# Jabruson/FDN-TIP2025

Measured on AMD Instinct MI355X. Metric: images/sec, FDN (LPNet->FDN forward) 1280x720 bs=8 fp32, higher is better.
Workload: dtype f32; 1 GPU; BASELINE.json configs[1]: FDN 1280x720 (padded 1280x736) batch=8 per GPU fp32; global_batch=8, parallelism=batch-shard x1, weights=synthetic (tamed 0.03) FDN + real LPNet, hip_streams=1, rccl_ranks=1, hip_graph=True, fdsa_full=False, fdsa_pair=False, no_tail_pin=False, tail_pin_l2=False, narrow_pipe=False, unfused_mlps=False, stats_launches=False, resample_upsample=False, aff_resized=False

## Files before the change

fdn-tip2025_amd/csrc/fdsa_tail.hpp:

```cpp
#pragma once
#include "common.hpp"

namespace {

constexpr int TL_SC1 = 16;

template <bool FULL, typename T>
__device__ __forceinline__ T tl_sq_acc(T q, T dl, bool live) {
#pragma clang fp contract(off)
    const T p = dl * dl;
    if constexpr (FULL) return q + p;
    else return q + (live ? p : T(0.f));
}

__host__ __device__ constexpr int tl_image_floats(int SH, int MT) { return ((6 * 2 * SH + 3 * 2 * SH * (MT * 32 + 1) + 255) / 256) * 256; }

__host__ __device__ constexpr int tl_image_floats_px1_c(int SH, int MT) { return 512 + 3 * ((SH + 7) / 8) * MT * 3 * 64 * 4; }
struct TailIo {
    const float* scr;
    const float* res;
    float* y;
    float* stats_out;
    int E, N, W, ty0, tx0;
    unsigned P;
    float* h;
    int Hd;
    int h_bf16;
    unsigned* ring_flag;
    int* ring_cnt;
};
__device__ __forceinline__ void tl_ring_release(const TailIo& io) {
    if (io.ring_flag && (threadIdx.x & 63) == 0) {
        if (__hip_atomic_fetch_add(io.ring_cnt, 1, __ATOMIC_RELAXED, __HIP_MEMORY_SCOPE_WORKGROUP) == 3)
            __hip_atomic_store(io.ring_flag, 0u, __ATOMIC_RELAXED, __HIP_MEMORY_SCOPE_AGENT);
    }
}

template <int SH, bool PIN = false, int NT = 3, bool FULL = false>
__device__ __forceinline__ void fdsa_tail_px2(const TailIo& io, const float* lds, const float* lds_pin = nullptr) {
    typedef fdn_f32x2 T;
    typedef fdn_f32x16 f32x16;
    constexpr int E2 = 2 * SH, WS = 33;
    const float* tg = lds;
    const float* tb = lds + 3 * E2;
    const float* Wl = lds + 6 * E2;
    const int E = io.E, N = io.N;
    const unsigned P = io.P, P4 = P * 4u;
    const int lane = threadIdx.x & 63, wave = threadIdx.x >> 6, kh = lane >> 5, ln = lane & 31;
    const int row = 2 * wave + (ln >> 4), col = 2 * (ln & 15);
    const bool ok = io.tx0 + col < io.W;
    const unsigned pix = (unsigned)((io.ty0 + row) * io.W + io.tx0 + col);
    constexpr unsigned PI = 1024u;
    const rsrc_t rg[3] = {mk_rsrc(io.scr, (unsigned)E * PI), mk_rsrc(io.scr + (long)E * 256, (unsigned)E * PI),
                          mk_rsrc(io.scr + (long)2 * E * 256, (unsigned)E * PI)};
    const rsrc_t rv = mk_rsrc(io.scr + (long)3 * E * 256, (unsigned)E * PI);
    const unsigned voff = kh * PI + (unsigned)(row * 32 + col) * 4u;
    const float invE = 1.0f / (float)E;

    T vv[SH], oa[SH], ob2[SH];
#pragma unroll
    for (int s = 0; s < SH; ++s) {
        vv[s] = bload2<TL_SC1>(rv, voff, (unsigned)(2 * s) * PI);
        oa[s] = bload2<TL_SC1>(rg[0], voff, (unsigned)(2 * s) * PI);
    }
    const unsigned nb4 = (unsigned)N * P4;
    const rsrc_t ro = mk_rsrc(io.y, nb4);
    const rsrc_t rr = mk_rsrc(io.res ? io.res : io.y, io.res ? nb4 : 0u);
    const unsigned vo = ok ? (4u * kh * P + pix) * 4u : 0x80000000u;
    T rres[16];
    f32x16 acc[2];
#pragma unroll
    for (int v = 0; v < 2; ++v)
#pragma unroll
        for (int r = 0; r < 16; ++r) acc[v][r] = 0.f;

#pragma unroll
    for (int g = 0; g < 3; ++g) {
        T* cur = (g & 1) ? ob2 : oa;
        if (g < 2) {
            T* nxt = (g & 1) ? oa : ob2;
#pragma unroll
            for (int s = 0; s < SH; ++s) nxt[s] = bload2<TL_SC1>(rg[g + 1], voff, (unsigned)(2 * s) * PI);
        }
        T m = 0.f;
#pragma unroll
        for (int s = 0; s < SH; ++s) m += cur[s];
        m = xsum32(m) * invE;
        T q = 0.f;
#pragma unroll
        for (int s = 0; s < SH; ++s) {
            const T dl = cur[s] - m;
            q = tl_sq_acc<FULL>(q, dl, 2 * s + kh < E);
        }
        const T rs = rsqrt_eps(xsum32(q) * invE);
#pragma unroll
        for (int s = 0; s < SH; ++s) {
            asm volatile("" ::: "memory");
            const int e = 2 * s + kh;
            cur[s] = ((cur[s] - m) * rs * tg[g * E2 + e] + tb[g * E2 + e]) * vv[s];
        }
        if (g == 2) {
            tl_ring_release(io);
#pragma unroll
            for (int r = 0; r < 16; ++r) {
                const fdn_u32x2 u = __builtin_amdgcn_raw_buffer_load_b64(rr, vo, (unsigned)((r & 3) + 8 * (r >> 2)) * P4, 0);
                rres[r] = T{__uint_as_float(u.x), __uint_as_float(u.y)};
            }
        }
#pragma unroll
        for (int s = 0; s < SH; ++s) {
            const float wa = Wl[(g * E2 + 2 * s + kh) * WS + ln];
            acc[0] = __builtin_amdgcn_mfma_f32_32x32x2f32(wa, cur[s].x, acc[0], 0, 0, 0);
            acc[1] = __builtin_amdgcn_mfma_f32_32x32x2f32(wa, cur[s].y, acc[1], 0, 0, 0);
        }
    }
    T outv[16];
    T sm = 0.f;
#pragma unroll
    for (int r = 0; r < 16; ++r) {
        const int nrow = (r & 3) + 8 * (r >> 2);
        T o = T{acc[0][r], acc[1][r]};
        o += rres[r];
        __builtin_amdgcn_raw_buffer_store_b64(fdn_u32x2{__float_as_uint(o.x), __float_as_uint(o.y)}, ro, vo, (unsigned)nrow * P4, 0);
        outv[r] = (FULL || nrow + 4 * kh < N) ? o : T(0.f);
        sm += outv[r];
    }
    if (io.stats_out || PIN) {
        T sq = 0.f;
        const T mean = xsum32(sm) / (float)N;
#pragma unroll
        for (int r = 0; r < 16; ++r) {
            const T dl = outv[r] - mean;
            sq = tl_sq_acc<FULL>(sq, dl, (r & 3) + 8 * (r >> 2) + 4 * kh < N);
        }
        const T rstd = rsqrt_eps(xsum32(sq) / (float)N);
        if (io.stats_out && kh == 0) {
            const rsrc_t rs_ = mk_rsrc(io.stats_out, 2u * P4);
            const unsigned vs = ok ? pix * 4u : 0x80000000u;
            __builtin_amdgcn_raw_buffer_store_b64(fdn_u32x2{__float_as_uint(mean.x), __float_as_uint(mean.y)}, rs_, vs, 0u, 0);
            __builtin_amdgcn_raw_buffer_store_b64(fdn_u32x2{__float_as_uint(rstd.x), __float_as_uint(rstd.y)}, rs_, vs, P4, 0);
        }
        if constexpr (PIN) {
            fdn_u32x4 Bf[2][2][3];
#pragma unroll
            for (int c = 0; c < 2; ++c) {
                const float sa = c ? rstd.y : rstd.x, sb = -(c ? mean.y : mean.x) * sa;
                float xn[16];
#pragma unroll
                for (int r = 0; r < 16; ++r) xn[r] = fmaf(c ? outv[r].y : outv[r].x, sa, sb);
#pragma unroll
                for (int ks = 0; ks < 2; ++ks) {
                    float v[8];
#pragma unroll
                    for (int b4 = 0; b4 < 4; ++b4) {
                        const auto sw = __builtin_amdgcn_permlane32_swap(__float_as_uint(xn[8 * ks + b4]), __float_as_uint(xn[8 * ks + 4 + b4]), false, false);
                        v[b4] = __uint_as_float(sw[0]);
                        v[4 + b4] = __uint_as_float(sw[1]);
                    }
#pragma unroll
                    for (int j = 0; j < 4; ++j) {
                        unsigned p1, p2, p3;
                        fdn_split3(v[2 * j], v[2 * j + 1], p1, p2, p3);
                        Bf[c][ks][0][j] = p1, Bf[c][ks][1][j] = p2, Bf[c][ks][2][j] = p3;
                    }
                }
            }
            const fdn_u32x4* wpin = reinterpret_cast<const fdn_u32x4*>(lds_pin) + lane;
            const float* bpin = lds_pin + NT * 2 * 3 * 64 * 4;
            const rsrc_t rh = mk_rsrc(io.h, (unsigned)io.Hd * P4);
            const unsigned vh = ok ? (4u * kh * P + pix) * 4u : 0x80000000u;
#pragma unroll
            for (int t = 0; t < NT; ++t) {
                f32x16 ah[2];
#pragma unroll
                for (int g = 0; g < 4; ++g) {
                    const float4 bv = *reinterpret_cast<const float4*>(&bpin[t * 32 + 8 * g + 4 * kh]);
#pragma unroll
                    for (int c = 0; c < 2; ++c) ah[c][4 * g] = bv.x, ah[c][4 * g + 1] = bv.y, ah[c][4 * g + 2] = bv.z, ah[c][4 * g + 3] = bv.w;
                }
#pragma unroll
                for (int ks = 0; ks < 2; ++ks) {
                    const fdn_u32x4 a3[3] = {wpin[((t * 2 + ks) * 3 + 0) * 64], wpin[((t * 2 + ks) * 3 + 1) * 64], wpin[((t * 2 + ks) * 3 + 2) * 64]};
                    ah[0] = fdn_mfma_split6(a3, Bf[0][ks], ah[0]);
                    ah[1] = fdn_mfma_split6(a3, Bf[1][ks], ah[1]);
                }
                if (io.h_bf16) {
                    const rsrc_t rhb = mk_rsrc(io.h, (unsigned)io.Hd * P * 2u);
                    const unsigned vhb = ok ? (4u * kh * P + pix) * 2u : 0x80000000u;
#pragma unroll
                    for (int r = 0; r < 16; ++r)
                        __builtin_amdgcn_raw_buffer_store_b32(pack_bf16(ah[0][r], ah[1][r]), rhb, vhb, (unsigned)(t * 32 + (r & 3) + 8 * (r >> 2)) * P * 2u, 0);
                } else {
#pragma unroll
                    for (int r = 0; r < 16; ++r)
                        __builtin_amdgcn_raw_buffer_store_b64(fdn_u32x2{__float_as_uint(ah[0][r]), __float_as_uint(ah[1][r])}, rh, vh,
                                                              (unsigned)(t * 32 + (r & 3) + 8 * (r >> 2)) * P4, 0);
                }
            }
        }
    }
}

#define FDN_TAIL_FN __forceinline__
typedef __attribute__((address_space(3))) const float* lds_cf;
typedef __attribute__((address_space(3))) const fdn_u32x4* lds_cu4;
template <int SH, int MT, bool FULL = false, bool PIN = false, int NT = 6>
__device__ FDN_TAIL_FN void fdsa_tail_px1(const TailIo& io, lds_cf tg, lds_cf tb, lds_cu4 W0, lds_cu4 W1, const float* gimg) {
    typedef fdn_f32x16 f32x16;
    constexpr int E2 = 2 * SH, NQ = (SH + 7) / 8;
    const int E = io.E, N = io.N;
    const unsigned P = io.P, P4 = P * 4u;
    const int lane = threadIdx.x & 63, wave = threadIdx.x >> 6, kh = lane >> 5, ln = lane & 31;
    constexpr unsigned PI = 1024u;
    const rsrc_t rg[3] = {mk_rsrc(io.scr, (unsigned)E * PI), mk_rsrc(io.scr + (long)E * 256, (unsigned)E * PI),
                          mk_rsrc(io.scr + (long)2 * E * 256, (unsigned)E * PI)};
    const rsrc_t rv = mk_rsrc(io.scr + (long)3 * E * 256, (unsigned)E * PI);
    const rsrc_t rw2 = mk_rsrc(gimg + 512 + 2 * NQ * MT * 3 * 64 * 4, (unsigned)(NQ * MT * 3 * 64) * 16u);
    const float invE = 1.0f / (float)E;
    const unsigned nb4 = (unsigned)N * P4;
    const rsrc_t ro = mk_rsrc(io.y, nb4);
    const rsrc_t rr = mk_rsrc(io.res ? io.res : io.y, io.res ? nb4 : 0u);
    const bool ok = io.tx0 + ln < io.W;

    float vv[SH], buf[2][SH];
    auto voff_of = [&](int rnd) { return kh * PI + (unsigned)((2 * wave + rnd) * 32 + ln) * 4u; };
    {
        const unsigned voff = voff_of(0);
        unsigned PIl = PI;
        asm volatile("" : "+s"(PIl));
#pragma unroll
        for (int s = 0; s < SH; ++s) {
            vv[s] = bload<TL_SC1>(rv, voff, (unsigned)(2 * s) * PIl);
            buf[0][s] = bload<TL_SC1>(rg[0], voff, (unsigned)(2 * s) * PIl);
        }
    }
#pragma unroll
    for (int rnd = 0; rnd < 2; ++rnd) {
        unsigned P4l = P4;
        asm volatile("" : "+s"(P4l));
        int khl = kh;
        asm volatile("" : "+v"(khl));
        const unsigned voff = voff_of(rnd);
        const unsigned pix = (unsigned)((io.ty0 + 2 * wave + rnd) * io.W + io.tx0 + ln);
        const unsigned vo = ok ? (4u * kh * P + pix) * 4u : 0x80000000u;
        f32x16 acc[MT];
#pragma unroll
        for (int mt = 0; mt < MT; ++mt)
#pragma unroll
            for (int r = 0; r < 16; ++r) acc[mt][r] = 0.f;
        float rres[MT][16];
#pragma unroll
        for (int g = 0; g < 3; ++g) {
            float* cur = buf[(rnd + g) & 1];
            float* nxt = buf[(rnd + g + 1) & 1];
            unsigned PIl = PI;
            asm volatile("" : "+s"(PIl));
            if (g < 2) {
#pragma unroll
                for (int s = 0; s < SH; ++s) nxt[s] = bload<TL_SC1>(rg[g + 1], voff, (unsigned)(2 * s) * PIl);
            }
// ... 153 lines not shown
```

fdn-tip2025_amd/csrc/patchfft.hip:

```cpp
#include "patch_fft.hpp"
#include "fdsa_tail.hpp"
#include <type_traits>

namespace {

constexpr int HS = 65 + 2;
constexpr int HALO = (TH + 2) * (TW + 2);
constexpr int HPT = (HALO + 255) / 256;

__device__ __forceinline__ void halo_offsets(int H, int W, int y0, int x0, unsigned (&goff)[HPT], int (&slot)[HPT]) {
#pragma unroll
    for (int i = 0; i < HPT; ++i) {
        const int idx = threadIdx.x + 256 * i;
        const int rr = idx / (TW + 2), cc = idx - rr * (TW + 2);
        const int y = y0 - 1 + rr, x = x0 - 1 + cc;
        const bool ok = idx < HALO && y >= 0 && y < H && x >= 0 && x < W;
        goff[i] = ok ? (unsigned)(y * W + x) * 4u : OOB;
        slot[i] = idx < HALO ? rr * HS + cc : (TH + 2) * HS;
    }
}
__device__ __forceinline__ void halo_fetch(rsrc_t r, unsigned plane_off, const unsigned (&goff)[HPT], float (&v)[HPT]) {
#pragma unroll
    for (int i = 0; i < HPT; ++i) v[i] = bload(r, goff[i], plane_off);
}
// ... 419 lines not shown
            }
            fft8<true>(z);
            constexpr float sc = 1.0f / 64.0f;
#pragma unroll
            for (int i = 0; i < 8; ++i) S[pj * PS + kx * KXS + i] = make_float2(z[i].x * sc, z[i].y * sc);
        }
        __syncthreads();

        if (more) build_filter();
        {
            float2 xk[5];
#pragma unroll
            for (int kx = 0; kx < 5; ++kx) xk[kx] = S[patch * PS + kx * KXS + rr];
            float r[8];
            irfft8_row(xk, r);
            float sp[8];
            second_conv(sp);
#pragma unroll
            for (int j = 0; j < 8; ++j) r[j] += sp[j];
            st_store8<OBF>(r, rout, ooff, (unsigned)__builtin_amdgcn_readfirstlane((int)((unsigned)c * hwo)));
        }
        __syncthreads();
    }
}


constexpr int FT_H = 8, FT_W = 32;
constexpr int FHW = FT_W + 2, FHH = FT_H + 2;
constexpr int FHP = FHH * FHW;
constexpr int FNS = (FHP + 31) / 32;
constexpr int FRS = 35;
constexpr int FPL = FHH * FRS;
constexpr int FEG = 8;
using f32x16 = fdn_f32x16;

struct FusedArgs {
    const float* x;
    long xbs;
    const float* stats;
    const float* wpk;
    const float* dww;
    const float* fftw;
    float* out;
    int E, H, W, tiles_x, tiles_per_img, nchunks;
    const float* tw;
    const float* res;
    float* y;
    float* stats_out;
    int N;
    float* h;
    int Hd, h_bf16;
};
constexpr int FDN_RING_CUS = 2048;
constexpr int FDN_RING_SLOTS = 2 * FDN_RING_CUS;
constexpr int FDN_RING_HDR = 16384;

template <int C, bool LN, bool OBF, int TAIL = 0>
__global__ __launch_bounds__(256, 2) void fdsa_fused_kernel(FusedArgs a) {
    static_assert(!TAIL || !OBF, "the in-kernel tail reads fp32 planes");
    constexpr bool CELLS = (C + 15) / 16 <= 2;
    __shared__ __attribute__((aligned(16))) float hid[32 * FPL];
    __shared__ __attribute__((aligned(16))) float2 S[3 * NP * PS];
    __shared__ __attribute__((aligned(16))) float wks[32 * 9];
    __shared__ __attribute__((aligned(16))) float fgs[FEG * 40];

    const int tid = threadIdx.x, lane = tid & 63, wave = tid >> 6, kh = lane >> 5, ln = lane & 31;
    const int t_ = (int)xcd_contiguous(blockIdx.x, gridDim.x);
    const int b = t_ / a.tiles_per_img, ti = t_ - b * a.tiles_per_img;
    const int ty0 = (ti / a.tiles_x) * FT_H, tx0 = (ti % a.tiles_x) * FT_W;
    const int E = a.E, H = a.H, W = a.W;
    const unsigned P = (unsigned)H * W, hw4 = P * 4u;
    const rsrc_t rx = mk_rsrc(a.x + (long)b * a.xbs, (unsigned)C * hw4);
    const rsrc_t rst = mk_rsrc(LN ? a.stats + (long)b * 2 * P : a.x, LN ? 2u * hw4 : 0u);
    constexpr unsigned OES = st_bytes<OBF>();
    const unsigned hwo = TAIL ? 1024u : P * OES;
    const float* scr_tile = a.out + (long)t_ * 4 * E * 256;
    rsrc_t rout = TAIL ? mk_rsrc(scr_tile, 4u * E * 1024u)
                       : mk_rsrc(reinterpret_cast<const float*>(reinterpret_cast<const char*>(a.out) + (long)b * 4 * E * P * OES), 4u * E * hwo);

    __shared__ int ring_s[4];
    if constexpr (TAIL != 0) {
        if (tid == 0) {
            unsigned hwid, xcc;
            asm volatile("s_getreg_b32 %0, hwreg(HW_REG_HW_ID)" : "=s"(hwid));
            asm volatile("s_getreg_b32 %0, hwreg(HW_REG_XCC_ID)" : "=s"(xcc));
            const unsigned cu = ((xcc & 7u) << 8) | (((hwid >> 13) & 7u) << 5) | (((hwid >> 12) & 1u) << 4) | ((hwid >> 8) & 0xFu);
            unsigned* f = reinterpret_cast<unsigned*>(a.out) + 2 * cu;
            int got = -1;
            while (got < 0) {
                const unsigned o0 = __hip_atomic_exchange(f, 1u, __ATOMIC_RELAXED, __HIP_MEMORY_SCOPE_AGENT);
                const unsigned o1 = __hip_atomic_exchange(f + 1, 1u, __ATOMIC_RELAXED, __HIP_MEMORY_SCOPE_AGENT);
                if (o0 == 0) {
                    got = 0;
                    if (o1 == 0) __hip_atomic_store(f + 1, 0u, __ATOMIC_RELAXED, __HIP_MEMORY_SCOPE_AGENT);
                } else if (o1 == 0) {
                    got = 1;
                } else {
                    __builtin_amdgcn_s_sleep(8);
                }
            }
            ring_s[0] = (int)(2 * cu) + got;
            ring_s[1] = 0;
            const unsigned long long blk = reinterpret_cast<unsigned long long>(a.out + FDN_RING_HDR + (long)(2 * cu + got) * (4 * a.E * 256));
            ring_s[2] = (int)(unsigned)blk;
            ring_s[3] = (int)(unsigned)(blk >> 32);
        }
    }
    constexpr int KST = (C + 15) / 16;
    fdn_u32x4 xb[3][KST][3];
    unsigned onebits = 0;
    int pixoff[3];
#pragma unroll
    for (int si = 0; si < 3; ++si) {
        const int s = wave + 4 * si;
        const int p = s * 32 + ln;
        const int r = p / FHW, c = p - r * FHW;
        const int gy = ty0 - 1 + r, gx = tx0 - 1 + c;
        const bool in_tile = s < FNS && p < FHP;
        const bool ok = in_tile && gy >= 0 && gy < H && gx >= 0 && gx < W;
        onebits |= (ok && kh == 0) ? (1u << si) : 0u;
        pixoff[si] = in_tile ? r * FRS + c : FHW;
        const unsigned g = ok ? (unsigned)(gy * W + gx) * 4u : OOB;
        float mu = 0.f, rs = 1.f;
        if (LN) {
            mu = bload(rst, g, 0);
            rs = bload(rst, g, hw4);
        }
        float xs[KST][8];
#pragma unroll
        for (int ks = 0; ks < KST; ++ks)
#pragma unroll
            for (int j = 0; j < 8; ++j) xs[ks][j] = bload(rx, g + (unsigned)(8 * kh) * hw4, (unsigned)(16 * ks + j) * hw4);
#pragma unroll
        for (int ks = 0; ks < KST; ++ks)
#pragma unroll
            for (int j = 0; j < 4; ++j) {
                float v0 = xs[ks][2 * j], v1 = xs[ks][2 * j + 1];
                if (LN) v0 = (v0 - mu) * rs, v1 = (v1 - mu) * rs;
                unsigned p1, p2, p3;
                fdn_split3(v0, v1, p1, p2, p3);
                xb[si][ks][0][j] = p1, xb[si][ks][1][j] = p2, xb[si][ks][2][j] = p3;
            }
    }

    const int el = wave * 2 + kh;
    const int row = lane & 7, px = (lane >> 3) & 3;
    const int slot = el * 4 + px;
    const int gx0 = tx0 + px * 8;
    const unsigned opix = TAIL ? (unsigned)(row * 32 + px * 8) * 4u : gx0 < W ? (unsigned)((ty0 + row) * W + gx0) * OES : OOB;
    const float* hb = hid + el * FPL + row * FRS + px * 8;

    constexpr int KS = KST * 3 + 1;
    constexpr bool AW_AHEAD = KS <= 7;
    fdn_u32x4 aw[AW_AHEAD ? KS : 1];
    auto aw_fetch = [&](int ch) {
        const fdn_u32x4* wp = reinterpret_cast<const fdn_u32x4*>(a.wpk) + ((long)ch * KS) * 64 + lane;
#pragma unroll
        for (int j = 0; j < (AW_AHEAD ? KS : 1); ++j) aw[j] = wp[j * 64];
    };
    float st_w = 0.f, st_w1 = 0.f, st_f0 = 0.f, st_f1 = 0.f;
    const rsrc_t rdw = mk_rsrc(a.dww, (unsigned)(4 * E * 9) * 4u), rfw = mk_rsrc(a.fftw, (unsigned)(E * 40) * 4u);
    auto stage_fetch = [&](int ch) {
        const int tid_o = tid;
        const int tid = [&] {
            if constexpr (KST >= 4 || TAIL == 3) { int t = threadIdx.x; asm volatile("" : "+v"(t)); return t; }
            else return tid_o;
        }();
        auto tap_of = [&](int i) {
            if constexpr (CELLS) {
                const int cl = i / 36, rem = i - cl * 36;
                const int ew = ch * FEG + cl;
                return bload(rdw, (unsigned)(((rem & 3) * E + (ew < E ? ew : E - 1)) * 9 + (rem >> 2)) * 4u, 0);
            }
            const int m = i / 9, tap = i - m * 9;
            const int ew = ch * FEG + (m & 7);
            return bload(rdw, (unsigned)(((m >> 3) * E + (ew < E ? ew : E - 1)) * 9 + tap) * 4u, 0);
        };
        st_w = tap_of(tid);
        st_w1 = tid < 32 ? tap_of(tid + 256) : 0.f;
        const int c0 = tid / 40, c1 = (tid + 256) / 40;
        const int e0_ = ch * FEG + c0, e1_ = ch * FEG + c1;
        st_f0 = bload(rfw, (unsigned)((e0_ < E ? e0_ : E - 1) * 40 + (tid - c0 * 40)) * 4u, 0);
        st_f1 = (tid < 64) ? bload(rfw, (unsigned)((e1_ < E ? e1_ : E - 1) * 40 + (tid + 256 - c1 * 40)) * 4u, 0) : 0.f;
    };
    auto stage_store = [&]() {
        wks[tid] = st_w;
        if (tid < 32) wks[tid + 256] = st_w1;
        fgs[tid] = st_f0;
        if (tid < 64) fgs[tid + 256] = st_f1;
    };
    auto mfma_phase = [&](int ch) __attribute__((always_inline)) {
        const fdn_u32x4* wp_ = reinterpret_cast<const fdn_u32x4*>(a.wpk) + ((long)ch * KS) * 64 + lane;
        int po[3];
        if constexpr (KST >= 4) {
            int t = threadIdx.x;
            asm volatile("" : "+v"(t));
#pragma unroll
            for (int si = 0; si < 3; ++si) {
                const int p = ((t >> 6) + 4 * si) * 32 + (t & 31);
                const int r = p / FHW, c = p - r * FHW;
                po[si] = p < FHP ? r * FRS + c : FHW;
            }
        } else {
#pragma unroll
            for (int si = 0; si < 3; ++si) po[si] = pixoff[si];
        }
#pragma unroll
        for (int si = 0; si < 3; ++si) {
            if (wave + 4 * si < FNS) {
                f32x16 acc;
#pragma unroll
                for (int r = 0; r < 16; ++r) acc[r] = 0.f;
#pragma unroll
                for (int ks = 0; ks < KST; ++ks) {
                    const fdn_u32x4 a3[3] = {AW_AHEAD ? aw[3 * ks] : wp_[(3 * ks) * 64], AW_AHEAD ? aw[3 * ks + 1] : wp_[(3 * ks + 1) * 64],
                                             AW_AHEAD ? aw[3 * ks + 2] : wp_[(3 * ks + 2) * 64]};
                    acc = fdn_mfma_split6(a3, xb[si][ks], acc);
                }
                const bool one = (onebits >> si) & 1u;
                const fdn_u32x4 xone = {one ? 0x3F803F80u : 0u, one ? 0x00003F80u : 0u, 0u, 0u};
                acc = fdn_mfma_bf16(AW_AHEAD ? aw[KS - 1] : wp_[(KS - 1) * 64], xone, acc);
                if constexpr (CELLS) {
#pragma unroll
                    for (int g = 0; g < 4; ++g)
                        reinterpret_cast<f32x4*>(hid)[(2 * g + kh) * FPL + po[si]] = f32x4{acc[4 * g], acc[4 * g + 1], acc[4 * g + 2], acc[4 * g + 3]};
                } else {
#pragma unroll
                    for (int r = 0; r < 16; ++r) hid[((r & 3) * 8 + 2 * (r >> 2) + kh) * FPL + po[si]] = acc[r];
                }
            }
        }
        if (AW_AHEAD && ch + 1 < a.nchunks) aw_fetch(ch + 1);
    };
    if (AW_AHEAD) aw_fetch(0);
    stage_fetch(0);
    stage_store();
    for (int ch = 0; ch < a.nchunks; ++ch) {
        const int e0 = ch * FEG;
        const int e = e0 + el;
        const bool more = ch + 1 < a.nchunks;
        mfma_phase(ch);
        if (more) stage_fetch(ch + 1);
        __syncthreads();
        if constexpr (TAIL != 0) {
            scr_tile = reinterpret_cast<const float*>(((unsigned long long)(unsigned)__builtin_amdgcn_readfirstlane(ring_s[3]) << 32) |
                                                      (unsigned)__builtin_amdgcn_readfirstlane(ring_s[2]));
            rout = mk_rsrc(scr_tile, 4u * E * 1024u);
        }

        auto dw_row8 = [&](const float* hp, const float* wk9, float (&o8)[8]) __attribute__((always_inline)) {
            float wkt[9];
#pragma unroll
            for (int i = 0; i < 9; ++i) wkt[i] = wk9[i];
#pragma unroll
            for (int j = 0; j < 8; ++j) o8[j] = 0.f;
#pragma unroll
            for (int dy = 0; dy < 3; ++dy) {
                float v[10];
#pragma unroll
                for (int j = 0; j < 10; ++j) v[j] = hp[dy * FRS + j];
#pragma unroll
                for (int j = 0; j < 8; ++j)
#pragma unroll
                    for (int dx = 0; dx < 3; ++dx) o8[j] = fmaf(wkt[dy * 3 + dx], v[j + dx], o8[j]);
            }
        };
        if constexpr (CELLS) {
            const f32x4* hc = reinterpret_cast<const f32x4*>(hid) + el * FPL + row * FRS + px * 8;
            f32x4 wk4[9];
#pragma unroll
            for (int i = 0; i < 9; ++i) wk4[i] = reinterpret_cast<const f32x4*>(wks)[el * 9 + i];
            fdn_f32x2 aqk[8], avv[8];
#pragma unroll
            for (int j = 0; j < 8; ++j) aqk[j] = fdn_f32x2{0.f, 0.f}, avv[j] = fdn_f32x2{0.f, 0.f};
#pragma unroll
            for (int dy = 0; dy < 3; ++dy) {
                f32x4 v[10];
#pragma unroll
                for (int j = 0; j < 10; ++j) v[j] = hc[dy * FRS + j];
#pragma unroll
                for (int j = 0; j < 8; ++j)
#pragma unroll
                    for (int dx = 0; dx < 3; ++dx) {
                        aqk[j] = __builtin_elementwise_fma(wk4[dy * 3 + dx].xy, v[j + dx].xy, aqk[j]);
                        avv[j] = __builtin_elementwise_fma(wk4[dy * 3 + dx].zw, v[j + dx].zw, avv[j]);
                    }
            }
#pragma unroll
            for (int t = 0; t < 3; ++t) {
                float o8[8];
#pragma unroll
                for (int j = 0; j < 8; ++j) o8[j] = t == 0 ? aqk[j].x : t == 1 ? aqk[j].y : avv[j].x;
                float2 sp[5];
                rfft8_row(o8, sp);
#pragma unroll
                for (int kx = 0; kx < 5; ++kx) S[(t * NP + slot) * PS + kx * KXS + row] = sp[kx];
            }
            float vv8[8];
#pragma unroll
            for (int j = 0; j < 8; ++j) vv8[j] = avv[j].y;
            st_store8<OBF>(vv8, rout, e < E ? opix + (unsigned)(3 * E + e) * hwo : OOB, 0);
        } else {
#pragma unroll
            for (int t = 0; t < 3; ++t) {
                float o8[8];
                dw_row8(hb + t * 8 * FPL, wks + (t * 8 + el) * 9, o8);
                float2 sp[5];
                rfft8_row(o8, sp);
#pragma unroll
                for (int kx = 0; kx < 5; ++kx) S[(t * NP + slot) * PS + kx * KXS + row] = sp[kx];
            }
        }
        __syncthreads();

        if (tid < NP * 5) {
            const int pj = tid / 5, kx = tid - pj * 5;
            float fg[8];
#pragma unroll
            for (int ky = 0; ky < 8; ++ky) fg[ky] = fgs[(pj >> 2) * 40 + ky * 5 + kx];
            constexpr float sc = 1.0f / 64.0f;
            float2 u_[8], v1_[8];
            float qka_[8], g_[8], va_[8];
            auto column = [&](auto as_written) __attribute__((always_inline)) {
                constexpr bool AW = decltype(as_written)::value;
                float2 q[8], k[8], v[8];
#pragma unroll
                for (int i = 0; i < 8; ++i) {
                    q[i] = S[(0 * NP + pj) * PS + kx * KXS + i];
                    k[i] = S[(1 * NP + pj) * PS + kx * KXS + i];
                    v[i] = S[(2 * NP + pj) * PS + kx * KXS + i];
                }
                fft8<false>(q);
                if (KST >= 4) __builtin_amdgcn_sched_barrier(0);
                fft8<false>(k);
                if (KST >= 4) __builtin_amdgcn_sched_barrier(0);
                fft8<false>(v);
                if (KST >= 4) __builtin_amdgcn_sched_barrier(0);
                float m = 1.0f;
#pragma unroll
                for (int ky = 0; ky < 8; ++ky) {
                    if (ky % 4 == 0) fdsa_bin<AW, true>(q[ky], k[ky], v[ky], fg[ky], m, u_[ky], v1_[ky], qka_[ky], g_[ky], va_[ky]);
                    else fdsa_bin<AW, false>(q[ky], k[ky], v[ky], fg[ky], m, u_[ky], v1_[ky], qka_[ky], g_[ky], va_[ky]);
                    if (KST >= 4) __builtin_amdgcn_sched_barrier(0);
                }
                return m;
            };
            if constexpr (KST >= 4) column(std::true_type{});
            else if (__builtin_amdgcn_ballot_w64(column(std::false_type{}) < 1e-10f) != 0) column(std::true_type{});
            if constexpr (KST >= 4) {
#pragma unroll
                for (int t = 0; t < 3; ++t) {
                    float2 o[8];
#pragma unroll
                    for (int ky = 0; ky < 8; ++ky)
                        o[ky] = t == 0 ? make_float2(va_[ky] * u_[ky].x, va_[ky] * u_[ky].y)
                              : t == 1 ? make_float2(g_[ky] * v1_[ky].x, g_[ky] * v1_[ky].y)
                                       : make_float2(qka_[ky] * u_[ky].x, qka_[ky] * u_[ky].y);
                    fft8<true>(o);
#pragma unroll
                    for (int i = 0; i < 8; ++i) S[(t * NP + pj) * PS + kx * KXS + i] = make_float2(o[i].x * sc, o[i].y * sc);
                    __builtin_amdgcn_sched_barrier(0);
                }
            } else {
                float2 o1[8], o2[8], o3[8];
#pragma unroll
                for (int ky = 0; ky < 8; ++ky) {
                    o1[ky] = make_float2(va_[ky] * u_[ky].x, va_[ky] * u_[ky].y);
                    o2[ky] = make_float2(g_[ky] * v1_[ky].x, g_[ky] * v1_[ky].y);
                    o3[ky] = make_float2(qka_[ky] * u_[ky].x, qka_[ky] * u_[ky].y);
                }
                fft8<true>(o1);
                fft8<true>(o2);
                fft8<true>(o3);
#pragma unroll
                for (int i = 0; i < 8; ++i) {
                    S[(0 * NP + pj) * PS + kx * KXS + i] = make_float2(o1[i].x * sc, o1[i].y * sc);
                    S[(1 * NP + pj) * PS + kx * KXS + i] = make_float2(o2[i].x * sc, o2[i].y * sc);
                    S[(2 * NP + pj) * PS + kx * KXS + i] = make_float2(o3[i].x * sc, o3[i].y * sc);
                }
            }
        } else if (!CELLS && wave == 3) {
            int t3 = threadIdx.x;
            if constexpr (KST >= 4) asm volatile("" : "+v"(t3));
            const int row3 = t3 & 7, px3 = (t3 >> 3) & 3, kh3 = (t3 >> 5) & 1;
#pragma unroll 1
            for (int i = 0; i < 4; ++i) {
                const int elv = 2 * i + (KST >= 4 ? kh3 : kh), ev = e0 + elv;
                float o8[8];
                dw_row8(hid + (24 + elv) * FPL + (KST >= 4 ? row3 * FRS + px3 * 8 : row * FRS + px * 8), wks + (24 + elv) * 9, o8);
                st_store8<OBF>(o8, rout, ev < E ? opix + (unsigned)(3 * E + ev) * hwo : OOB, 0);
            }
        }
        __syncthreads();

#pragma unroll
        for (int t = 0; t < 3; ++t) {
            float2 xk[5];
#pragma unroll
            for (int kx = 0; kx < 5; ++kx) xk[kx] = S[(t * NP + slot) * PS + kx * KXS + row];
            float r8[8];
            irfft8_row(xk, r8);
            st_store8<OBF>(r8, rout, e < E ? opix + (unsigned)(t * E + e) * hwo : OOB, 0);
        }
        if (more) stage_store();
    }
    if constexpr (TAIL == 1 || TAIL == 3) {
        constexpr int SH = 19;
        constexpr bool PIN = TAIL == 3;
        constexpr int NBLK0 = tl_image_floats(SH, 1) / 256;
        constexpr int NBLK = NBLK0 + (PIN ? tl_pin_floats(3) / 256 : 0);
        const rsrc_t rtw = mk_rsrc(a.tw, (unsigned)NBLK * 1024u);
#pragma unroll
        for (int i = 0; i < (NBLK + 3) / 4; ++i) {
            const int blk = __builtin_amdgcn_readfirstlane(wave + 4 * i);
            if (blk < NBLK)
                __builtin_amdgcn_raw_ptr_buffer_load_lds(rtw, (__attribute__((address_space(3))) void*)(hid + blk * 256), 16, (unsigned)(blk * 1024 + lane * 16), 0, 0, 0);
        }
        asm volatile("s_waitcnt vmcnt(0)" ::: "memory");
        __syncthreads();
        TailIo io;
        io.scr = scr_tile;
        io.res = a.res ? a.res + (long)b * a.N * P : nullptr;
        io.y = a.y + (long)b * a.N * P;
        io.stats_out = a.stats_out ? a.stats_out + (long)b * 2 * P : nullptr;
        io.E = E; io.N = a.N; io.W = W; io.ty0 = ty0; io.tx0 = tx0; io.P = P;
        io.h = PIN ? reinterpret_cast<float*>(reinterpret_cast<char*>(a.h) + (long)b * a.Hd * P * (a.h_bf16 ? 2 : 4)) : nullptr;
        io.Hd = a.Hd;
        io.h_bf16 = a.h_bf16;
        io.ring_flag = reinterpret_cast<unsigned*>(a.out) + ring_s[0];
        io.ring_cnt = ring_s + 1;
        constexpr bool FULL = C == 32;
        fdsa_tail_px2<SH, PIN, 3, FULL>(io, hid, hid + NBLK0 * 256);
    }
    if constexpr (TAIL == 2 || TAIL == 4) {
        constexpr int SH = 38, MT = 2, NQ = (SH + 7) / 8, GB = NQ * MT * 3;
        constexpr bool PIN2 = TAIL == 4;
        const rsrc_t rtw = mk_rsrc(a.tw, (unsigned)tl_image_floats_px1(SH, MT) * 4u);
        auto dma = [&](const void* dst, int src_blk, int nblk, int first = -1) {
            for (int i = first < 0 ? wave : (wave - first) & 3; i < nblk; i += 4) {
                const int blk = __builtin_amdgcn_readfirstlane(i);
                __builtin_amdgcn_raw_ptr_buffer_load_lds(rtw, (__attribute__((address_space(3))) void*)(reinterpret_cast<const char*>(dst) + blk * 1024), 16,
                                                         (unsigned)((src_blk + blk) * 1024 + lane * 16), 0, 0, 0);
            }
        };
        dma(wks, 0, 1, 2);
        dma(fgs, 1, 1, 3);
        dma(hid, 2, GB);
        asm volatile("s_waitcnt vmcnt(0)" ::: "memory");
        __syncthreads();
        dma(S, 2 + GB, GB);
        TailIo io;
        io.scr = scr_tile;
        io.res = a.res ? a.res + (long)b * a.N * P : nullptr;
        io.y = a.y + (long)b * a.N * P;
        io.stats_out = a.stats_out ? a.stats_out + (long)b * 2 * P : nullptr;
        io.E = E; io.N = a.N; io.W = W; io.ty0 = ty0; io.tx0 = tx0; io.P = P;
        io.h = PIN2 ? a.h + (long)b * a.Hd * P : nullptr;
        io.Hd = a.Hd;
        io.h_bf16 = 0;
        io.ring_flag = reinterpret_cast<unsigned*>(a.out) + ring_s[0];
        io.ring_cnt = ring_s + 1;
        fdsa_tail_px1<SH, MT, C == 64, PIN2>(io, (lds_cf)wks, (lds_cf)fgs, (lds_cu4)hid, (lds_cu4)S, a.tw);
    }
}

__global__ void fdsa_tail_pack_kernel(const float* __restrict__ w, const float* __restrict__ gamma, const float* __restrict__ beta, float* __restrict__ img,
                                      int E, int N, int SH, int MT, int total) {
    const int i = blockIdx.x * blockDim.x + threadIdx.x;
    if (i >= total) return;
    const int E2 = 2 * SH, WS = MT * 32 + 1;
    float v = 0.f;
    if (i < 6 * E2) {
        const int j = i < 3 * E2 ? i : i - 3 * E2;
        const int g = j / E2, e = j - g * E2;
        if (e < E) v = (i < 3 * E2 ? gamma : beta)[g * E + e];
    } else if (i < 6 * E2 + 3 * E2 * WS) {
        const int j = i - 6 * E2;
        const int k = j / WS, n = j - k * WS;
        const int g = k / E2, e = k - g * E2;
        if (n < N && e < E) v = w[(long)n * 3 * E + g * E + e];
    }
    img[i] = v;
}

__global__ void fdsa_pack_kernel(const float* __restrict__ w, const float* __restrict__ gamma, const float* __restrict__ beta,
                                 fdn_u32x4* __restrict__ wpk, int C, int E, int nchunks, int channel_major) {
    const int idx = blockIdx.x * blockDim.x + threadIdx.x;
    const int KST = (C + 15) / 16, KS = KST * 3 + 1;
    if (idx >= nchunks * KS * 64) return;
    const int lane = idx & 63, j = (idx >> 6) % KS, ch = (idx >> 6) / KS;
    const int m = lane & 31, kh = lane >> 5;
    const int e = ch * FEG + (channel_major ? m >> 2 : m & 7), kind = channel_major ? m & 3 : m >> 3;
    auto part_of = [](float x, int part) {
        for (int p = 0; p < part; ++p) x -= __uint_as_float(__float_as_uint(x) & 0xffff0000u);
        return __float_as_uint(x) >> 16;
    };
    fdn_u32x4 o = {0u, 0u, 0u, 0u};
    if (e < E) {
        const float* wr = w + (long)(kind * E + e) * C;
        if (j < KS - 1) {
            const int ks = j / 3, part = j - 3 * ks;
#pragma unroll
            for (int q = 0; q < 4; ++q) {
                unsigned hl[2];
#pragma unroll
                for (int u = 0; u < 2; ++u) {
                    const int k = 16 * ks + 8 * kh + 2 * q + u;
                    float v = k < C ? wr[k] : 0.f;
                    if (gamma && k < C) v *= gamma[k];
                    hl[u] = part_of(v, part);
                }
                o[q] = hl[0] | (hl[1] << 16);
            }
        } else if (kh == 0 && beta) {
            double sacc = 0.0;
            for (int k = 0; k < C; ++k) sacc += (double)wr[k] * (double)beta[k];
            const float bsum = (float)sacc;
            o[0] = part_of(bsum, 0) | (part_of(bsum, 1) << 16);
            o[1] = part_of(bsum, 2);
        }
    }
    wpk[idx] = o;
}

}

extern "C" int fdn_fdsa_core(const float* hidden, const float* dw_w, const float* fft_w, float* out, int B, int E, int H,
                             int W, fdn_stream_t stream) {
    FDN_CHECK_ARG(hidden && dw_w && fft_w && out && B > 0 && E > 0 && H > 0 && W > 0);
    FDN_CHECK_ARG(H % 8 == 0 && W % 8 == 0 && E < 65536 && B < 65536);
    FDN_CHECK_ARG((reinterpret_cast<uintptr_t>(out) & 15) == 0);
    FDN_CHECK_ARG(16ull * E * H * W < 0x80000000ull);
    const int tx = cdiv(W, TW), ty = cdiv(H, TH);
    const int cus = fdn_device_cus();
    if (cus <= 0) return FDN_ERR_LAUNCH;
    const long want = 8L * 3 * cus, per = (long)tx * ty * B;
    long groups = (want + per - 1) / per;
    groups = groups < 1 ? 1 : (groups > E ? E : groups);
    int EPB = (int)((E + groups - 1) / groups);
    if (EPB > 8) EPB = 8;
    const int ngrp = (E + EPB - 1) / EPB;
    if (W % 4 == 0 && (reinterpret_cast<uintptr_t>(hidden) & 15) == 0)
        hipLaunchKernelGGL(fdsa_core_kernel<true>, dim3((unsigned)(tx * ty) * ngrp * B), dim3(256), 0, static_cast<hipStream_t>(stream), hidden, dw_w,
                           fft_w, out, E, H, W, tx, tx * ty, EPB);
    else
        hipLaunchKernelGGL(fdsa_core_kernel<false>, dim3((unsigned)(tx * ty) * ngrp * B), dim3(256), 0, static_cast<hipStream_t>(stream), hidden, dw_w,
                           fft_w, out, E, H, W, tx, tx * ty, EPB);
    return fdn_launch_status();
}

extern "C" int fdn_fdffn_mid(const void* x_, const float* w0, const float* w2, const float* ffta, const float* fftp,
                             void* out_, int B, int Hd, int H, int W, int x_bf16, int out_bf16, fdn_stream_t stream) {
    const float* x = static_cast<const float*>(x_);
    float* out = static_cast<float*>(out_);
// ... 234 lines not shown
```

Measured before the change: 28.45 images/s.

## Prefetch MFMA weights late via buffer loads and skip dead tail-chunk waves

For kernels with many k-steps (where weights were previously read from global memory inside the MFMA loop), the weight fragments are now prefetched into registers with buffer loads after the second barrier of each chunk, so the next chunk's loads overlap the inverse-FFT stage. Waves whose channel slots fall beyond E in the last partial chunk now skip the depthwise, FFT-column and irfft work, and the spectral column threads and the wave-3 loop are limited to live channels. A scheduling barrier is added after the residual loads in the tail kernel. The larger register array for weights raises register pressure in the KST>=4 variants and may reduce occupancy.

```diff
diff --git a/fdn-tip2025_amd/csrc/fdsa_tail.hpp b/fdn-tip2025_amd/csrc/fdsa_tail.hpp
--- a/fdn-tip2025_amd/csrc/fdsa_tail.hpp
+++ b/fdn-tip2025_amd/csrc/fdsa_tail.hpp
@@ -106,6 +106,7 @@
                 const fdn_u32x2 u = __builtin_amdgcn_raw_buffer_load_b64(rr, vo, (unsigned)((r & 3) + 8 * (r >> 2)) * P4, 0);
                 rres[r] = T{__uint_as_float(u.x), __uint_as_float(u.y)};
             }
+            __builtin_amdgcn_sched_barrier(0);
         }
 #pragma unroll
         for (int s = 0; s < SH; ++s) {
diff --git a/fdn-tip2025_amd/csrc/patchfft.hip b/fdn-tip2025_amd/csrc/patchfft.hip
--- a/fdn-tip2025_amd/csrc/patchfft.hip
+++ b/fdn-tip2025_amd/csrc/patchfft.hip
@@ -595,11 +595,16 @@
 
     constexpr int KS = KST * 3 + 1;
     constexpr bool AW_AHEAD = KS <= 7;
-    fdn_u32x4 aw[AW_AHEAD ? KS : 1];
+    fdn_u32x4 aw[KS];
+    const rsrc_t rwp = mk_rsrc(a.wpk, (unsigned)(a.nchunks * KS) * 1024u);
+    auto aw_fetch_late = [&](int ch) {
+#pragma unroll
+        for (int j = 0; j < KS; ++j) aw[j] = __builtin_amdgcn_raw_buffer_load_b128(rwp, (unsigned)lane * 16u, (unsigned)((ch * KS + j) * 1024), 0);
+    };
     auto aw_fetch = [&](int ch) {
         const fdn_u32x4* wp = reinterpret_cast<const fdn_u32x4*>(a.wpk) + ((long)ch * KS) * 64 + lane;
 #pragma unroll
-        for (int j = 0; j < (AW_AHEAD ? KS : 1); ++j) aw[j] = wp[j * 64];
+        for (int j = 0; j < KS; ++j) aw[j] = wp[j * 64];
     };
     float st_w = 0.f, st_w1 = 0.f, st_f0 = 0.f, st_f1 = 0.f;
     const rsrc_t rdw = mk_rsrc(a.dww, (unsigned)(4 * E * 9) * 4u), rfw = mk_rsrc(a.fftw, (unsigned)(E * 40) * 4u);
@@ -633,7 +638,6 @@
         if (tid < 64) fgs[tid + 256] = st_f1;
     };
     auto mfma_phase = [&](int ch) __attribute__((always_inline)) {
-        const fdn_u32x4* wp_ = reinterpret_cast<const fdn_u32x4*>(a.wpk) + ((long)ch * KS) * 64 + lane;
         int po[3];
         if constexpr (KST >= 4) {
             int t = threadIdx.x;
@@ -656,13 +660,12 @@
                 for (int r = 0; r < 16; ++r) acc[r] = 0.f;
 #pragma unroll
                 for (int ks = 0; ks < KST; ++ks) {
-                    const fdn_u32x4 a3[3] = {AW_AHEAD ? aw[3 * ks] : wp_[(3 * ks) * 64], AW_AHEAD ? aw[3 * ks + 1] : wp_[(3 * ks + 1) * 64],
-                                             AW_AHEAD ? aw[3 * ks + 2] : wp_[(3 * ks + 2) * 64]};
+                    const fdn_u32x4 a3[3] = {aw[3 * ks], aw[3 * ks + 1], aw[3 * ks + 2]};
                     acc = fdn_mfma_split6(a3, xb[si][ks], acc);
                 }
                 const bool one = (onebits >> si) & 1u;
                 const fdn_u32x4 xone = {one ? 0x3F803F80u : 0u, one ? 0x00003F80u : 0u, 0u, 0u};
-                acc = fdn_mfma_bf16(AW_AHEAD ? aw[KS - 1] : wp_[(KS - 1) * 64], xone, acc);
+                acc = fdn_mfma_bf16(aw[KS - 1], xone, acc);
                 if constexpr (CELLS) {
 #pragma unroll
                     for (int g = 0; g < 4; ++g)
@@ -676,12 +679,15 @@
         if (AW_AHEAD && ch + 1 < a.nchunks) aw_fetch(ch + 1);
     };
     if (AW_AHEAD) aw_fetch(0);
+    if (!AW_AHEAD) aw_fetch_late(0);
     stage_fetch(0);
     stage_store();
     for (int ch = 0; ch < a.nchunks; ++ch) {
         const int e0 = ch * FEG;
         const int e = e0 + el;
         const bool more = ch + 1 < a.nchunks;
+        const int live = E - e0;
+        const bool wave_live = 2 * __builtin_amdgcn_readfirstlane(wave) < live;
         mfma_phase(ch);
         if (more) stage_fetch(ch + 1);
         __syncthreads();
@@ -708,7 +714,9 @@
                     for (int dx = 0; dx < 3; ++dx) o8[j] = fmaf(wkt[dy * 3 + dx], v[j + dx], o8[j]);
             }
         };
-        if constexpr (CELLS) {
+        float vv8[8] = {0.f, 0.f, 0.f, 0.f, 0.f, 0.f, 0.f, 0.f};
+        if (!wave_live) {
+        } else if constexpr (CELLS) {
             const f32x4* hc = reinterpret_cast<const f32x4*>(hid) + el * FPL + row * FRS + px * 8;
             f32x4 wk4[9];
 #pragma unroll
@@ -739,10 +747,8 @@
 #pragma unroll
                 for (int kx = 0; kx < 5; ++kx) S[(t * NP + slot) * PS + kx * KXS + row] = sp[kx];
             }
-            float vv8[8];
 #pragma unroll
             for (int j = 0; j < 8; ++j) vv8[j] = avv[j].y;
-            st_store8<OBF>(vv8, rout, e < E ? opix + (unsigned)(3 * E + e) * hwo : OOB, 0);
         } else {
 #pragma unroll
             for (int t = 0; t < 3; ++t) {
@@ -754,9 +760,10 @@
                 for (int kx = 0; kx < 5; ++kx) S[(t * NP + slot) * PS + kx * KXS + row] = sp[kx];
             }
         }
+        if constexpr (CELLS) st_store8<OBF>(vv8, rout, e < E ? opix + (unsigned)(3 * E + e) * hwo : OOB, 0);
         __syncthreads();
 
-        if (tid < NP * 5) {
+        if (tid < (live < FEG ? live : FEG) * 20) {
             const int pj = tid / 5, kx = tid - pj * 5;
             float fg[8];
 #pragma unroll
@@ -827,7 +834,7 @@
             if constexpr (KST >= 4) asm volatile("" : "+v"(t3));
             const int row3 = t3 & 7, px3 = (t3 >> 3) & 3, kh3 = (t3 >> 5) & 1;
 #pragma unroll 1
-            for (int i = 0; i < 4; ++i) {
+            for (int i = 0; i < 4 && 2 * i < live; ++i) {
                 const int elv = 2 * i + (KST >= 4 ? kh3 : kh), ev = e0 + elv;
                 float o8[8];
                 dw_row8(hid + (24 + elv) * FPL + (KST >= 4 ? row3 * FRS + px3 * 8 : row * FRS + px * 8), wks + (24 + elv) * 9, o8);
@@ -836,13 +843,16 @@
         }
         __syncthreads();
 
+        if (!AW_AHEAD) aw_fetch_late(ch + 1);
 #pragma unroll
         for (int t = 0; t < 3; ++t) {
-            float2 xk[5];
-#pragma unroll
-            for (int kx = 0; kx < 5; ++kx) xk[kx] = S[(t * NP + slot) * PS + kx * KXS + row];
-            float r8[8];
-            irfft8_row(xk, r8);
+            float r8[8] = {0.f, 0.f, 0.f, 0.f, 0.f, 0.f, 0.f, 0.f};
+            if (wave_live) {
+                float2 xk[5];
+#pragma unroll
+                for (int kx = 0; kx < 5; ++kx) xk[kx] = S[(t * NP + slot) * PS + kx * KXS + row];
+                irfft8_row(xk, r8);
+            }
             st_store8<OBF>(r8, rout, e < E ? opix + (unsigned)(t * E + e) * hwo : OOB, 0);
         }
         if (more) stage_store();
```

After: 28.59 images/s (median of 6 runs). No clear change (+0.5%).
